# zsyOAOA/ResShift

Hardware: NVIDIA H100
Metric: 256x256 x4 SR images/sec (15 steps), denoising hot path (higher is better)
Workload: dtype f16 (fp32 accumulate)

## Files before the change

resshift_b200/csrc/common.cuh:

```cuda
#pragma once

#include <cuda.h>
#include <cuda_fp16.h>
#include <cuda_runtime.h>
#include <cstdint>
#include <cstdio>
#include <string>

namespace rs {

void set_error(const std::string& msg);
int fail(int code, const std::string& msg);

#define RS_CUDA_OK(expr)                                                                       \
  do {                                                                                         \
    cudaError_t _e = (expr);                                                                   \
    if (_e != cudaSuccess) {                                                                   \
      (void)cudaGetLastError();             \
      return ::rs::fail(-2, std::string(#expr) + " failed: " + cudaGetErrorString(_e) + " (" + \
                                __FILE__ + ":" + std::to_string(__LINE__) + ")");              \
    }                                                                                          \
  } while (0)

#define RS_CHECK(cond, msg)                                                              \
  do {                                                                                   \
    if (!(cond)) {                                                                       \
      return ::rs::fail(-1, std::string("check failed: ") + #cond + " — " + (msg) + " (" + \
                                __FILE__ + ":" + std::to_string(__LINE__) + ")");        \
    }                                                                                    \
  } while (0)

#ifdef __CUDACC__

__device__ __forceinline__ uint32_t smem_u32(const void* p) {
  return static_cast<uint32_t>(__cvta_generic_to_shared(p));
}

__device__ __forceinline__ bool elect_one() {
  uint32_t pred = 0;
  asm volatile(
      "{\n\t"
      ".reg .pred P;\n\t"
      "elect.sync _|P, 0xffffffff;\n\t"
      "selp.u32 %0, 1, 0, P;\n\t"
      "}\n"
      : "=r"(pred));
  return pred != 0;
}

__device__ __forceinline__ void pdl_wait() { asm volatile("griddepcontrol.wait;" ::: "memory"); }
__device__ __forceinline__ void pdl_trigger() { asm volatile("griddepcontrol.launch_dependents;" ::: "memory"); }

__device__ __forceinline__ float silu_f(float v) { return __fdividef(v, 1.0f + __expf(-v)); }
__device__ __forceinline__ float gelu_erf_f(float v) {
  const float z = fminf(fabsf(v) * 0.70710678118654752f, 4.0f);
  float pz = fmaf(z, -2.177763781e-05f, 5.068330793e-04f);
  pz = fmaf(z, pz, -5.339398049e-03f);
  pz = fmaf(z, pz, 3.423144668e-02f);
  pz = fmaf(z, pz, -1.528908461e-01f);
  pz = fmaf(z, pz, -9.167589545e-01f);
  pz = fmaf(z, pz, -1.628154397e+00f);
  pz = fmaf(z, pz, 6.178960575e-06f);
  float ex;
  asm("ex2.approx.ftz.f32 %0, %1;" : "=f"(ex) : "f"(pz));
  const float h = 0.5f * v;
  return h + fmaf(-fabsf(h), ex, fabsf(h));
}

__device__ __forceinline__ void mbar_init(uint64_t* bar, uint32_t count) {
  asm volatile("mbarrier.init.shared::cta.b64 [%0], %1;" ::"r"(smem_u32(bar)), "r"(count));
}
__device__ __forceinline__ void mbar_fence_init() {
  asm volatile("fence.mbarrier_init.release.cluster;" ::: "memory");
}
__device__ __forceinline__ void mbar_arrive_expect_tx(uint64_t* bar, uint32_t bytes) {
  asm volatile("mbarrier.arrive.expect_tx.shared::cta.b64 _, [%0], %1;" ::"r"(smem_u32(bar)), "r"(bytes)
               : "memory");
}
__device__ __forceinline__ void mbar_arrive(uint64_t* bar) {
  asm volatile("mbarrier.arrive.shared::cta.b64 _, [%0];" ::"r"(smem_u32(bar)) : "memory");
}
__device__ __forceinline__ bool mbar_try_wait(uint64_t* bar, uint32_t parity) {
  uint32_t ok;
  asm volatile(
      "{\n\t"
      ".reg .pred P;\n\t"
      "mbarrier.try_wait.parity.shared::cta.b64 P, [%1], %2;\n\t"
      "selp.u32 %0, 1, 0, P;\n\t"
      "}\n"
      : "=r"(ok)
      : "r"(smem_u32(bar)), "r"(parity)
      : "memory");
  return ok != 0;
}
__device__ __forceinline__ void mbar_arrive_remote(uint32_t bar_cluster_addr) {
  asm volatile("mbarrier.arrive.shared::cluster.b64 _, [%0];" ::"r"(bar_cluster_addr) : "memory");
}
__device__ __forceinline__ uint64_t global_timer_ns() {
  uint64_t t;
  asm volatile("mov.u64 %0, %%globaltimer;" : "=l"(t));
  return t;
}
__device__ __forceinline__ void mbar_wait(uint64_t* bar, uint32_t parity) {
  if (mbar_try_wait(bar, parity)) return;
  const uint64_t t0 = global_timer_ns();
  uint32_t spins = 0;
  while (!mbar_try_wait(bar, parity)) {
    if ((++spins & 0xFFu) == 0 && global_timer_ns() - t0 > 2000000000ull) __trap();
  }
}

__device__ __forceinline__ void tma_prefetch_desc(const CUtensorMap* m) {
  asm volatile("prefetch.tensormap [%0];" ::"l"(reinterpret_cast<uint64_t>(m)) : "memory");
}
__device__ __forceinline__ void tma_load_2d(void* dst, const CUtensorMap* m, uint64_t* bar, int c0, int c1) {
  asm volatile(
      "cp.async.bulk.tensor.2d.shared::cluster.global.tile.mbarrier::complete_tx::bytes [%0], [%1, {%3, %4}], [%2];"
      ::"r"(smem_u32(dst)), "l"(reinterpret_cast<uint64_t>(m)), "r"(smem_u32(bar)), "r"(c0), "r"(c1)
      : "memory");
}
__device__ __forceinline__ void tma_load_4d(void* dst, const CUtensorMap* m, uint64_t* bar, int c0, int c1, int c2,
                                            int c3) {
  asm volatile(
      "cp.async.bulk.tensor.4d.shared::cluster.global.tile.mbarrier::complete_tx::bytes [%0], [%1, {%3, %4, %5, %6}], "
      "[%2];" ::"r"(smem_u32(dst)),
      "l"(reinterpret_cast<uint64_t>(m)), "r"(smem_u32(bar)), "r"(c0), "r"(c1), "r"(c2), "r"(c3)
      : "memory");
}

__device__ __forceinline__ uint32_t cluster_ctarank() {
  uint32_t r;
  asm volatile("mov.u32 %0, %%cluster_ctarank;" : "=r"(r));
  return r;
}
__device__ __forceinline__ void cluster_sync_all() {
  asm volatile("barrier.cluster.arrive.release.aligned;" ::: "memory");
  asm volatile("barrier.cluster.wait.acquire.aligned;" ::: "memory");
}
__device__ __forceinline__ uint32_t mapa_u32(uint32_t addr, uint32_t rank) {
  uint32_t r;
  asm volatile("mapa.shared::cluster.u32 %0, %1, %2;" : "=r"(r) : "r"(addr), "r"(rank));
  return r;
}
__device__ __forceinline__ void tma_load_2d_mc(void* dst, const CUtensorMap* m, uint64_t* bar, int c0, int c1, uint16_t cta_mask) {
  asm volatile(
      "cp.async.bulk.tensor.2d.shared::cluster.global.tile.mbarrier::complete_tx::bytes.multicast::cluster [%0], [%1, {%3, %4}], [%2], %5;"
      ::"r"(smem_u32(dst)), "l"(reinterpret_cast<uint64_t>(m)), "r"(smem_u32(bar)), "r"(c0), "r"(c1), "h"(cta_mask)
      : "memory");
}

__device__ __forceinline__ void tma_store_4d(const CUtensorMap* m, const void* src, int c0, int c1, int c2, int c3) {
  asm volatile("cp.async.bulk.tensor.4d.global.shared::cta.tile.bulk_group [%0, {%2, %3, %4, %5}], [%1];" ::"l"(
                   reinterpret_cast<uint64_t>(m)),
               "r"(smem_u32(src)), "r"(c0), "r"(c1), "r"(c2), "r"(c3)
               : "memory");
}
__device__ __forceinline__ void tma_store_commit() { asm volatile("cp.async.bulk.commit_group;" ::: "memory"); }
__device__ __forceinline__ void tma_store_wait_read() { asm volatile("cp.async.bulk.wait_group.read 0;" ::: "memory"); }
__device__ __forceinline__ void tma_store_wait_read_keep1() { asm volatile("cp.async.bulk.wait_group.read 1;" ::: "memory"); }
__device__ __forceinline__ void st_shared_v4(uint32_t addr, uint32_t a, uint32_t b, uint32_t c, uint32_t d) {
  asm volatile("st.shared.v4.b32 [%0], {%1, %2, %3, %4};" ::"r"(addr), "r"(a), "r"(b), "r"(c), "r"(d) : "memory");
}
__device__ __forceinline__ void fence_proxy_async_smem() { asm volatile("fence.proxy.async.shared::cta;" ::: "memory"); }
__device__ __forceinline__ void named_bar_sync(int id, int nthreads) {
  asm volatile("bar.sync %0, %1;" ::"r"(id), "r"(nthreads) : "memory");
}

__device__ __forceinline__ void wgmma_fence() { asm volatile("wgmma.fence.sync.aligned;" ::: "memory"); }
__device__ __forceinline__ void wgmma_commit() { asm volatile("wgmma.commit_group.sync.aligned;" ::: "memory"); }
template <int kPending>
__device__ __forceinline__ void wgmma_wait() { asm volatile("wgmma.wait_group.sync.aligned %0;" ::"n"(kPending) : "memory"); }
template <int kRegs>
__device__ __forceinline__ void wgmma_fence_regs(float (&d)[kRegs]) {
#pragma unroll
  for (int i = 0; i < kRegs; ++i) asm volatile("" : "+f"(d[i])::"memory");
}

__device__ __forceinline__ uint64_t wgmma_desc_sw128(uint32_t smem_addr) {
  uint64_t d = 0;
  d |= static_cast<uint64_t>((smem_addr & 0x3FFFFu) >> 4);
  d |= static_cast<uint64_t>(1) << 16;
  d |= static_cast<uint64_t>(1024 >> 4) << 32;
  d |= static_cast<uint64_t>(1) << 62;
  return d;
}

#endif

}
```

resshift_b200/csrc/gn_stats.cuh:

```cuda
#pragma once

#include "common.cuh"

namespace rs {

struct GnSink {
  float* part;
  float* gstat;
  unsigned int* counter;
  int cstride;
  int coff;
  unsigned int expected;
  float eps;
};

#ifdef __CUDACC__

__device__ __forceinline__ float2 ldcg_f2(const float* p) {
  float2 v;
  asm volatile("ld.global.cg.v2.f32 {%0, %1}, [%2];" : "=f"(v.x), "=f"(v.y) : "l"(p) : "memory");
  return v;
}

__device__ __forceinline__ unsigned int atom_add_acq_rel_gpu(unsigned int* p, unsigned int v) {
  unsigned int old;
  asm volatile("atom.add.acq_rel.gpu.global.u32 %0, [%1], %2;" : "=r"(old) : "l"(p), "r"(v) : "memory");
  return old;
}

__device__ __forceinline__ void chan_merge_equal(float n, float m0, float q0, float m1, float q1, float& m, float& q) {
  m = 0.5f * (m0 + m1);
  const float d0 = m0 - m, d1 = m1 - m;
  q = q0 + q1 + n * (d0 * d0 + d1 * d1);
}

template <int kG>
__device__ __forceinline__ void gn_finalize_groups(const float* part, int n, int slots, int C, int g0, int gstep, int cpg, float ns,
                                                   float eps, float* gstat, int lane) {
  const float* base = part + (size_t)n * slots * C * 2;
  const int K = slots * cpg;
  float pivot[kG], s1[kG], s2[kG];
#pragma unroll
  for (int q = 0; q < kG; ++q) {
    const int g = g0 + q * gstep;
    pivot[q] = g < 32 ? ldcg_f2(base + (size_t)(g * cpg) * 2).x : 0.f;
    s1[q] = 0.f; s2[q] = 0.f;
  }
  for (int i0 = 0; i0 < K; i0 += 128) {
    float2 e[kG][4];
#pragma unroll
    for (int q = 0; q < kG; ++q) {
      const int g = g0 + q * gstep;
#pragma unroll
      for (int u = 0; u < 4; ++u) {
        const int i = i0 + u * 32 + lane;
        if (g < 32 && i < K) {
          const int sl = i / cpg, c = i - sl * cpg;
          e[q][u] = ldcg_f2(base + ((size_t)sl * C + g * cpg + c) * 2);
        } else {
          e[q][u] = make_float2(pivot[q], 0.f);
        }
      }
    }
#pragma unroll
    for (int q = 0; q < kG; ++q)
#pragma unroll
      for (int u = 0; u < 4; ++u) {
        const float d = e[q][u].x - pivot[q];
        s1[q] += d;
        s2[q] += fmaf(ns * d, d, e[q][u].y);
      }
  }
#pragma unroll
  for (int q = 0; q < kG; ++q) {
    float a = s1[q], b = s2[q];
#pragma unroll
    for (int off = 16; off; off >>= 1) {
      a += __shfl_xor_sync(0xffffffffu, a, off);
      b += __shfl_xor_sync(0xffffffffu, b, off);
    }
    const int g = g0 + q * gstep;
    const float invK = 1.0f / (float)K;
    const float dm = a * invK;
    const float m2 = fmaxf(b - ns * (float)K * dm * dm, 0.f);
    const float var = m2 * invK / ns;
    if (lane == 0 && g < 32) {
      gstat[((size_t)n * 32 + g) * 2] = pivot[q] + dm;
      gstat[((size_t)n * 32 + g) * 2 + 1] = rsqrtf(var + eps);
    }
  }
}

template <int kMax>
__device__ __forceinline__ void gn_arrive(const GnSink* const (&sink)[kMax], const int (&img)[kMax], const unsigned int (&add)[kMax],
                                          int slots, float ns, int tid, int nthreads, int bar_id, int* s_flag ) {
  named_bar_sync(bar_id, nthreads);
  if (tid < kMax) {
    int last = 0;
    if (sink[tid] != nullptr && img[tid] >= 0 && sink[tid]->gstat != nullptr) {
      const unsigned int old = atom_add_acq_rel_gpu(sink[tid]->counter + img[tid], add[tid]);
      last = (old + add[tid] == sink[tid]->expected) ? 1 : 0;
    }
    s_flag[tid] = last;
  }
  named_bar_sync(bar_id, nthreads);
  const int warp = tid >> 5, lane = tid & 31, nwarps = nthreads >> 5;
#pragma unroll
  for (int i = 0; i < kMax; ++i) {
    if (!s_flag[i]) continue;
    const GnSink& s = *sink[i];
    const int cpg = s.cstride / 32;
    for (int g = warp; g < 32; g += 4 * nwarps) gn_finalize_groups<4>(s.part, img[i], slots, s.cstride, g, nwarps, cpg, ns, s.eps, s.gstat, lane);
  }
  named_bar_sync(bar_id, nthreads);
}

template <typename Ld>
__device__ __forceinline__ void pivot_stats2(Ld ld, int rows, float2& mean, float2& m2) {
  const float2 p = ld(0);
  float2 s1 = make_float2(0.f, 0.f), s2 = make_float2(0.f, 0.f);
  for (int r = 1; r < rows; ++r) {
    const float2 v = ld(r);
    const float dx = v.x - p.x, dy = v.y - p.y;
    s1.x += dx; s1.y += dy;
    s2.x = fmaf(dx, dx, s2.x); s2.y = fmaf(dy, dy, s2.y);
  }
  const float inv = 1.0f / (float)rows;
  mean = make_float2(p.x + s1.x * inv, p.y + s1.y * inv);
  m2 = make_float2(fmaxf(s2.x - s1.x * s1.x * inv, 0.f), fmaxf(s2.y - s1.y * s1.y * inv, 0.f));
}

__device__ __forceinline__ void warp_chunk_stats(const uint4& o0, const uint4& o1, int lane, float* dst) {
  float sv[16], sq[16];
  const __half2* q0 = reinterpret_cast<const __half2*>(&o0);
  const __half2* q1 = reinterpret_cast<const __half2*>(&o1);
#pragma unroll
  for (int j = 0; j < 4; ++j) {
    const float2 x0 = __half22float2(q0[j]);
    const float2 x1 = __half22float2(q1[j]);
    sv[2 * j] = x0.x; sv[2 * j + 1] = x0.y; sv[8 + 2 * j] = x1.x; sv[8 + 2 * j + 1] = x1.y;
  }
#pragma unroll
  for (int j = 0; j < 16; ++j) sq[j] = sv[j] * sv[j];
#pragma unroll
  for (int half = 8, bit = 16; half >= 1; half >>= 1, bit >>= 1) {
    const bool upper = (lane & bit) != 0;
#pragma unroll
    for (int j = 0; j < half; ++j) {
      const float send_s = upper ? sv[j] : sv[j + half];
      const float keep_s = upper ? sv[j + half] : sv[j];
      sv[j] = keep_s + __shfl_xor_sync(0xffffffffu, send_s, bit);
      const float send_q = upper ? sq[j] : sq[j + half];
      const float keep_q = upper ? sq[j + half] : sq[j];
      sq[j] = keep_q + __shfl_xor_sync(0xffffffffu, send_q, bit);
    }
  }
  sv[0] += __shfl_xor_sync(0xffffffffu, sv[0], 1);
  sq[0] += __shfl_xor_sync(0xffffffffu, sq[0], 1);
  if ((lane & 1) == 0) {
    const int cidx = ((lane >> 4) & 1) * 8 + ((lane >> 3) & 1) * 4 + ((lane >> 2) & 1) * 2 + ((lane >> 1) & 1);
    const float mean = sv[0] * (1.0f / 32.0f);
    dst[cidx * 2] = mean;
    dst[cidx * 2 + 1] = fmaxf(sq[0] - sv[0] * mean, 0.f);
  }
}

__device__ __forceinline__ void write_quad_pairs(const float* wq, int BN, int ncols, int col0, int bn, int n0, int Nimg, int slot,
                                                 int slots, const GnSink& s0, const GnSink& s1, int tid, int nthreads) {
  for (int cc = tid; cc < ncols; cc += nthreads) {
    float m[4], q[4];
#pragma unroll
    for (int k = 0; k < 4; ++k) { m[k] = wq[((size_t)k * BN + cc) * 2]; q[k] = wq[((size_t)k * BN + cc) * 2 + 1]; }
    float ma, qa, mb, qb;
    chan_merge_equal(32.f, m[0], q[0], m[1], q[1], ma, qa);
    chan_merge_equal(32.f, m[2], q[2], m[3], q[3], mb, qb);
#pragma unroll
    for (int d = 0; d < 2; ++d) {
      const GnSink& s = d == 0 ? s0 : s1;
      if (!s.part) continue;
      const size_t ch = (size_t)s.coff + col0 + cc;
      float* dst = s.part + (((size_t)n0 * slots + slot) * s.cstride + ch) * 2;
      if (bn == 1) {
        float mm, qq;
        chan_merge_equal(64.f, ma, qa, mb, qb, mm, qq);
        dst[0] = mm; dst[1] = qq;
      } else {
        dst[0] = ma; dst[1] = qa;
        if (n0 + 1 < Nimg) {
          float* dst1 = s.part + (((size_t)(n0 + 1) * slots + slot) * s.cstride + ch) * 2;
          dst1[0] = mb; dst1[1] = qb;
        }
      }
    }
  }
}

__device__ __forceinline__ float2 gn_channel_from_pairs(const float* part_nc , int slots, int C, float ns) {
  const float pivot = reinterpret_cast<const float2*>(part_nc)->x;
  float s1 = 0.f, s2 = 0.f;
  int sl = 0;
  for (; sl + 16 <= slots; sl += 16) {
    float2 e[16];
#pragma unroll
    for (int u = 0; u < 16; ++u) e[u] = *reinterpret_cast<const float2*>(part_nc + (size_t)(sl + u) * C * 2);
#pragma unroll
    for (int u = 0; u < 16; ++u) { const float d = e[u].x - pivot; s1 += d; s2 += fmaf(ns * d, d, e[u].y); }
  }
  for (; sl + 4 <= slots; sl += 4) {
    float2 e[4];
#pragma unroll
    for (int u = 0; u < 4; ++u) e[u] = *reinterpret_cast<const float2*>(part_nc + (size_t)(sl + u) * C * 2);
#pragma unroll
    for (int u = 0; u < 4; ++u) { const float d = e[u].x - pivot; s1 += d; s2 += fmaf(ns * d, d, e[u].y); }
  }
  for (; sl < slots; ++sl) {
    const float2 e = *reinterpret_cast<const float2*>(part_nc + (size_t)sl * C * 2);
    const float d = e.x - pivot; s1 += d; s2 += fmaf(ns * d, d, e.y);
  }
  const float dm = s1 / (float)slots;
  return make_float2(pivot + dm, fmaxf(s2 - ns * (float)slots * dm * dm, 0.f));
}
__device__ __forceinline__ float2 gn_group_from_channels(const float* ch_pairs , int cpg, float cnt, float eps) {
  const float pivot = ch_pairs[0];
  float s1 = 0.f, s2 = 0.f;
  for (int j = 0; j < cpg; ++j) { const float d = ch_pairs[2 * j] - pivot; s1 += d; s2 += fmaf(cnt * d, d, ch_pairs[2 * j + 1]); }
  const float dm = s1 / (float)cpg;
  const float m2 = fmaxf(s2 - cnt * (float)cpg * dm * dm, 0.f);
  return make_float2(pivot + dm, rsqrtf(m2 / (cnt * (float)cpg) + eps));
}

#endif
}
```

resshift_b200/csrc/launch.cuh:

```cuda
#pragma once

#include <algorithm>
#include <atomic>
#include <cstdlib>
#include <cmath>
#include <cstring>
#include <mutex>
#include <utility>
#include <vector>

#include "common.cuh"
#include "conv_gemm.cuh"
#include "elementwise.cuh"
#include "mlp_fused.cuh"
#include "norm_act.cuh"
#include "window_attn.cuh"
#include "swin_attn_fused.cuh"
#include "vq_attn.cuh"
#include "unet_attn.cuh"

namespace rs {

typedef CUresult (*PFN_encodeTiled)(CUtensorMap*, CUtensorMapDataType, cuuint32_t, void*, const cuuint64_t*,
                                    const cuuint64_t*, const cuuint32_t*, const cuuint32_t*, CUtensorMapInterleave,
// ... 464 lines not shown
    RS_CUDA_OK(cudaFuncSetAttribute(unet_attn_sm90_kernel<128>, cudaFuncAttributeMaxDynamicSharedMemorySize, UnetAttnSmem<128>::launch_bytes));
    attr_set[dev].store(true, std::memory_order_release);
  }
  return 0;
}

inline int conv_launch(const ConvDesc& d, cudaStream_t st) {
  if (d.simt_kernel) {
    const long long npix = (long long)d.prm.Nimg * d.prm.Hout * d.prm.Wout;
    const int warps = 8;
    (void)launch_k(conv_simt_kernel, dim3((unsigned)((npix + warps - 1) / warps)), dim3(warps * 32), (size_t)(0), st, d.prm, d.simt);
  } else {
    const ConvKernelFn k = conv_kernel_for(d.prm.BN, d.prm.msub, d.has_silu || d.film);
    RS_CHECK(k != nullptr, "no conv kernel for this channel tile");
    (void)launch_kc(k, dim3(d.grid), dim3(kConvThreads), (size_t)(d.smem), st, d.prm.cg, d.prm);
    if (d.prm.splitk > 1)
      (void)launch_k(splitk_reduce_kernel, dim3(d.red_grid_x, d.prm.Nimg, d.red_grid_z), dim3(256), d.red_smem, st, d.red);
  }
  RS_CUDA_OK(cudaGetLastError());
  return 0;
}

inline int conv_tile_slots(int H, int W, bool* fusable = nullptr) {
  const int bw = pow2_floor_div(W, kConvBM);
  const int bh = pow2_floor_div(H, kConvBM / bw);
  if (fusable) *fusable = (kConvBM / (bw * bh)) <= 2;
  return (W / bw) * (H / bh);
}

struct GnDesc {
  View in, out;
  const float* gamma = nullptr; const float* beta = nullptr;
  const float* film = nullptr; long long film_sN = 0;
  int film_off = -1;
  int silu = 0;
  float* part = nullptr;
  float* gstat = nullptr;
  unsigned int* counter = nullptr;
  float eps = 1e-5f;
  int slots = 0;
  bool fused = false;
  bool finalize_kernel = false;
};

inline void gn_chunks(int HW, int N, int* chunks, int* rows) {
  int c = std::max(1, std::min((HW + 31) / 32, (num_sms() * 4 + N - 1) / N));
  while (c > 1 && HW % c != 0) --c;
  *chunks = c; *rows = HW / c;
}

struct GnGeometry {
  int slots = 0;
  int rows_per_slot = 0;
  int stats_ctas = 0;
  bool finalize = false;
  int apply_ctas = 0;
  int apply_rows = 0;
  int csplit = 1;
};

inline GnGeometry gn_geometry(const GnDesc& g) {
  const int C = g.in.C, HW = g.in.H * g.in.W, N = g.in.N;
  GnGeometry r;
  r.slots = g.slots;
  if (!g.fused) {
    int chunks, rows;
    gn_chunks(HW, N, &chunks, &rows);
    if (r.slots <= 0) r.slots = chunks;
    r.stats_ctas = r.slots;
  }
  r.rows_per_slot = r.slots > 0 ? HW / r.slots : 0;
  r.finalize = g.fused && g.finalize_kernel;
  int actas = std::max(1, std::min((HW + 15) / 16, (num_sms() * 4 + N - 1) / N));
  r.apply_rows = (HW + actas - 1) / actas;
  r.apply_ctas = (HW + r.apply_rows - 1) / r.apply_rows;
  const int cpg = C / 32;
  int unit = cpg; while (unit % 8) unit += cpg;
  for (int cs = 2; r.apply_ctas * N * r.csplit < num_sms() * 3 / 2 && cs <= C / unit; ++cs)
    if (C % cs == 0 && (C / cs) % unit == 0) r.csplit = cs;
  return r;
}

inline int gn_launch(const GnDesc& g, cudaStream_t st) {
  const int C = g.in.C, HW = g.in.H * g.in.W, N = g.in.N;
  RS_CHECK(C % 32 == 0 && C % 8 == 0 && C <= 2048, "GroupNorm channel count");
  RS_CHECK(g.in.ld % 8 == 0 && g.out.ld % 8 == 0, "GroupNorm view alignment");
  RS_CHECK(g.gstat != nullptr || g.part != nullptr, "GroupNorm needs a statistics buffer");
  const GnGeometry geo = gn_geometry(g);
  const int slots = geo.slots;
  if (!g.fused) {
    const int lanes = 256 / (C / 8);
    RS_CHECK(g.part != nullptr && (g.gstat == nullptr || g.counter != nullptr), "GroupNorm statistics buffers");
    RS_CHECK(HW % slots == 0, "GroupNorm statistics slots must divide H*W");
    GnStatsParams sp{};
    sp.x = g.in.ptr; sp.sN = g.in.sN(); sp.ld = g.in.ld; sp.C = C; sp.HW = HW; sp.N = N;
    sp.sink.part = g.part; sp.sink.gstat = g.gstat; sp.sink.counter = g.counter; sp.sink.cstride = C; sp.sink.coff = 0;
    sp.sink.expected = (unsigned)(slots * C); sp.sink.eps = g.eps;
    sp.slots = slots; sp.rows_per_slot = geo.rows_per_slot;
    (void)launch_k(gn_stats_kernel, dim3(geo.stats_ctas, N), dim3(256), (size_t)lanes * C * 3 * sizeof(float) + 16, st, sp);
    RS_CUDA_OK(cudaGetLastError());
  }
  if (geo.finalize) {
    RS_CHECK(g.part != nullptr && g.gstat != nullptr && slots > 0 && HW % slots == 0, "GroupNorm finalisation buffers");
    GnFinalizeParams fp{g.part, g.gstat, slots, C, (float)geo.rows_per_slot, g.eps};
    (void)launch_k(gn_finalize_kernel, dim3(32, N), dim3(256), (size_t)0, st, fp);
    RS_CUDA_OK(cudaGetLastError());
  }
  GnApplyParams ap{g.in.ptr, g.in.sN(), g.in.ld, g.out.ptr, g.out.sN(), g.out.ld, C, HW, N, g.gstat, g.part, slots, g.eps,
                   g.gamma, g.beta, g.film, g.film_sN, g.silu, geo.apply_rows, C / geo.csplit};
  (void)launch_k(gn_apply_kernel, dim3(geo.apply_ctas, N, geo.csplit), dim3(256),
                 (size_t)(4 * (C / geo.csplit) + 64) * sizeof(float), st, ap);
  RS_CUDA_OK(cudaGetLastError());
  return 0;
}

struct MlpDesc {
  View in, out, res;
  bool has_res = true;
  const __half* w1 = nullptr; const float* b1 = nullptr;
  const __half* w2 = nullptr; const float* b2 = nullptr;
  int E = 0, Hd = 0;
  GnSink sink[2] = {};
  MlpParams prm;
  int grid = 0; size_t smem = 0;
};

inline bool mlp_supported(int E, int Hd, int H, int W, int N) {
  (void)N;
  bool fus = false;
  conv_tile_slots(H, W, &fus);
  return (E == 64 || E == 128 || E == 192 || E == 256) && Hd % kMlpHc == 0 && fus;
}

inline int mlp_finalize(MlpDesc& d) {
  MlpParams& p = d.prm;
  std::memset(&p, 0, sizeof(p));
  const int H = d.in.H, W = d.in.W, N = d.in.N;
  RS_CHECK(mlp_supported(d.E, d.Hd, H, W, N), "fused MLP: unsupported shape (E in {64, 128, 192, 256}, hidden % 64)");
  RS_CHECK(d.in.C == d.E && d.out.C == d.E, "fused MLP: channel mismatch");
  p.E = d.E; p.Hd = d.Hd; p.bias1 = d.b1; p.bias2 = d.b2;
  p.bw = pow2_floor_div(W, kConvBM);
  p.bh = pow2_floor_div(H, kConvBM / p.bw);
  p.bn = kConvBM / (p.bw * p.bh);
  p.tiles_w = W / p.bw; p.tiles_h = H / p.bh;
  const int tiles_n = (N + p.bn - 1) / p.bn;
  p.Wout = W; p.Hout = H; p.Nimg = N;
  const int slot = std::max(kMlpHc, d.E) * kConvBK * 2;
  const int fixed = MlpSmem(d.E, d.Hd, 0).total + 1024;
  p.ring = std::min(8, (227 * 1024 - fixed) / slot);
  RS_CHECK(p.ring >= 2, "fused MLP: not enough shared memory for the weight ring");
  d.smem = (size_t)MlpSmem(d.E, d.Hd, p.ring).total + 1024;
  RS_CHECK(d.smem <= 227 * 1024, "fused MLP: shared memory budget exceeded");
  p.has_res = d.has_res ? 1 : 0;
  d.grid = p.tiles_w * p.tiles_h * tiles_n;
  int rc = encode_act_map(&p.tmX, d.in.ptr, d.E, W, H, N, d.in.sW(), d.in.sH(), d.in.sN(), p.bw, p.bh, p.bn, 64);
  if (rc) return rc;
  rc = encode_weight_map(&p.tmW1, d.w1, d.E, d.Hd, kMlpHc); if (rc) return rc;
  rc = encode_weight_map(&p.tmW2, d.w2, d.Hd, d.E, d.E); if (rc) return rc;
  rc = encode_act_map(&p.tmOut, d.out.ptr, d.E, W, H, N, d.out.sW(), d.out.sH(), d.out.sN(), p.bw, p.bh, p.bn, 64);
  if (rc) return rc;
  if (d.has_res) {
    rc = encode_act_map(&p.tmRes, d.res.ptr, d.E, W, H, N, d.res.sW(), d.res.sH(), d.res.sN(), p.bw, p.bh, p.bn, 64);
    if (rc) return rc;
  }
  p.gn_slots = p.tiles_w * p.tiles_h;
  compact_sinks(d.sink, p.gn_slots, p.sink);
  return 0;
}

inline int mlp_launch(const MlpDesc& d, cudaStream_t st) {
  switch (d.E) {
    case 64: (void)launch_k(mlp_fused_sm90_kernel<64>, dim3(d.grid), dim3(kMlpThreads), d.smem, st, d.prm); break;
    case 128: (void)launch_k(mlp_fused_sm90_kernel<128>, dim3(d.grid), dim3(kMlpThreads), d.smem, st, d.prm); break;
    case 192: (void)launch_k(mlp_fused_sm90_kernel<192>, dim3(d.grid), dim3(kMlpThreads), d.smem, st, d.prm); break;
    case 256: (void)launch_k(mlp_fused_sm90_kernel<256>, dim3(d.grid), dim3(kMlpThreads), d.smem, st, d.prm); break;
    default: RS_CHECK(false, "fused MLP: embedding width");
  }
  RS_CUDA_OK(cudaGetLastError());
  return 0;
}

struct SwinAttnDesc {
  View x, y;
  int heads = 0, shift = 0;
  const float* gn_part = nullptr; int gn_slots = 0; const float* gn_gstat = nullptr;
  const float* gamma = nullptr; const float* beta = nullptr;
  const __half* wqkv = nullptr; int wqkv_ld = 0; const float* bqkv = nullptr;
  const float* relbias = nullptr;
  const __half* wproj = nullptr; int wproj_ld = 0; const float* bproj = nullptr;
  GnSink sink[2] = {};
  SwinAttnParams prm;
  GnFinalizeParams fin[2] = {};
  int grid = 0;
};
inline bool swin_attn_supported(int E, int heads, int H, int W, int window) {
  return window == 8 && (E == 192 || E == 64) && heads * 32 == E && H % 8 == 0 && W % 8 == 0;
}
inline int swin_attn_finalize(SwinAttnDesc& d) {
  SwinAttnParams& p = d.prm;
  std::memset(&p, 0, sizeof(p));
  const int E = d.x.C;
  RS_CHECK(swin_attn_supported(E, d.heads, d.x.H, d.x.W, 8), "fused Swin attention: E in {64, 192}, head_dim 32, H and W multiples of 8");
  RS_CHECK(d.y.C == E && d.y.H == d.x.H && d.y.W == d.x.W && d.y.N == d.x.N, "fused Swin attention: output geometry");
  RS_CHECK(d.x.ld % 8 == 0 && d.y.ld % 8 == 0 && d.wqkv_ld % 8 == 0 && d.wproj_ld % 8 == 0, "fused Swin attention: 16-byte rows");
  RS_CHECK((d.gn_part && d.gn_slots > 0) || d.gn_gstat, "fused Swin attention: norm1 statistics");
  int rc = encode_weight_map(&p.tmWqkv, d.wqkv, d.wqkv_ld, 3 * E, 64); if (rc) return rc;
  rc = encode_weight_map(&p.tmWproj, d.wproj, d.wproj_ld, E, 64); if (rc) return rc;
  p.x = d.x.ptr; p.x_ld = d.x.ld; p.y = d.y.ptr; p.y_ld = d.y.ld;
  p.N = d.x.N; p.H = d.x.H; p.W = d.x.W; p.heads = d.heads; p.shift = d.shift; p.scale = 0.17677669529663687f;
  p.gn_part = d.gn_part; p.gn_slots = d.gn_slots; p.gn_gstat = d.gn_gstat; p.gamma = d.gamma; p.beta = d.beta; p.eps = 1e-5f;
  p.wqkv = d.wqkv; p.wqkv_ld = d.wqkv_ld; p.bqkv = d.bqkv; p.relbias = d.relbias;
  p.wproj = d.wproj; p.wproj_ld = d.wproj_ld; p.bproj = d.bproj;
  p.total_windows = d.x.N * (d.x.H / 8) * (d.x.W / 8);
  const int nW = (d.x.H / 8) * (d.x.W / 8);
  compact_sinks(d.sink, nW, p.sink);
  const int pairs = (p.total_windows + 1) / 2;
  d.grid = std::min(pairs, num_sms());
  for (int k = 0; k < 2; ++k) {
    d.fin[k] = GnFinalizeParams{};
    if (p.sink[k].gstat) {
      RS_CHECK(p.sink[k].coff == 0 && p.sink[k].cstride == E, "fused Swin attention: group statistics of a channel slice");
      d.fin[k] = GnFinalizeParams{p.sink[k].part, p.sink[k].gstat, nW, E, 64.0f, p.sink[k].eps};
    }
    p.sink[k].gstat = nullptr; p.sink[k].counter = nullptr;
  }
  return 0;
}
inline int swin_attn_launch(const SwinAttnDesc& d, cudaStream_t st) {
  if (d.x.C == 192) (void)launch_k(swin_attn_fused_kernel<192>, dim3(d.grid), dim3(kSwinThreads), (size_t)SwinSmem<192>::launch_bytes, st, d.prm);
  else (void)launch_k(swin_attn_fused_kernel<64>, dim3(d.grid), dim3(kSwinThreads), (size_t)SwinSmem<64>::launch_bytes, st, d.prm);
  RS_CUDA_OK(cudaGetLastError());
  for (int k = 0; k < 2; ++k)
    if (d.fin[k].gstat) {
      (void)launch_k(gn_finalize_kernel, dim3(32, d.x.N), dim3(256), (size_t)0, st, d.fin[k]);
      RS_CUDA_OK(cudaGetLastError());
    }
  return 0;
}

struct VqAttnDesc {
  View q, k, v, out;
  int row_begin = 0, row_end = -1;
  VqAttnParams prm;
};
inline int vq_attn_set_rows(VqAttnDesc& d, long long row_begin, long long row_end, bool allow_empty) {
  const long long T = (long long)d.q.H * d.q.W;
  RS_CHECK(row_begin >= 0 && row_begin <= row_end && row_end <= T,
           "fused VQ-GAN attention: rows [" + std::to_string(row_begin) + ", " + std::to_string(row_end) + ") outside [0, T = " + std::to_string(T) + ")");
  RS_CHECK(row_begin % kVqAttnBM == 0 && row_end % kVqAttnBM == 0, "fused VQ-GAN attention: row range bounds must be multiples of 64");
  RS_CHECK(allow_empty || row_end > row_begin, "fused VQ-GAN attention: empty row range");
  d.row_begin = (int)row_begin; d.row_end = (int)row_end;
  d.prm.q_tile0 = (int)(row_begin / kVqAttnBM);
  return 0;
}
inline int vq_attn_finalize(VqAttnDesc& d) {
  VqAttnParams& p = d.prm;
  std::memset(&p, 0, sizeof(p));
  const int N = d.q.N, C = d.q.C;
  const long long T = (long long)d.q.H * d.q.W;
  RS_CHECK(C == 128 || C == 256 || C == 512, "fused VQ-GAN attention: C in {128, 256, 512}, got " + std::to_string(C));
  RS_CHECK(T > 0 && T % kVqAttnBM == 0 && T <= (1LL << 30), "fused VQ-GAN attention: T = H * W must be a positive multiple of 64, got " + std::to_string(T));
  RS_CHECK(N >= 1 && N <= 65535, "fused VQ-GAN attention: batch in [1, 65535]");
  const View* vs[4] = {&d.q, &d.k, &d.v, &d.out};
  for (const View* v : vs) {
    RS_CHECK(v->N == N && (long long)v->H * v->W == T && v->C == C, "fused VQ-GAN attention: q, k, v, out must all be [N, T, C]");
    RS_CHECK(v->ptr != nullptr && v->ld >= C && v->ld % 8 == 0, "fused VQ-GAN attention: rows of >= C elements, 16-byte aligned");
  }
  p.T = (int)T;
  { int rc = vq_attn_set_rows(d, d.row_begin, d.row_end < 0 ? T : d.row_end, true); if (rc) return rc; }
  p.scale_log2 = (float)(1.4426950408889634 / std::sqrt((double)C));
  CUtensorMap* maps[4] = {&p.tmQ, &p.tmK, &p.tmV, &p.tmO};
  const int rows[4] = {kVqAttnBM, vq_attn_bk(C), vq_attn_bk(C), kVqAttnBM};
  for (int i = 0; i < 4; ++i) {
    const View& v = *vs[i];
    int rc = encode_act_map(maps[i], v.ptr, C, (int)T, 1, N, v.ld, T * v.ld, v.sN(), rows[i], 1, 1, 64);
    if (rc) return rc;
  }
  return 0;
}
inline int vq_attn_launch(const VqAttnDesc& d, cudaStream_t st) {
  if (d.row_end == d.row_begin) return 0;
  const dim3 grid((unsigned)((d.row_end - d.row_begin) / kVqAttnBM), (unsigned)d.q.N);
  switch (d.q.C) {
    case 128: (void)launch_k(vq_attn_sm90_kernel<128>, grid, dim3(kVqAttnThreads), (size_t)VqAttnSmem<128>::launch_bytes, st, d.prm); break;
    case 256: (void)launch_k(vq_attn_sm90_kernel<256>, grid, dim3(kVqAttnThreads), (size_t)VqAttnSmem<256>::launch_bytes, st, d.prm); break;
    case 512: (void)launch_k(vq_attn_sm90_kernel<512>, grid, dim3(kVqAttnThreads), (size_t)VqAttnSmem<512>::launch_bytes, st, d.prm); break;
    default: RS_CHECK(false, "fused VQ-GAN attention: C in {128, 256, 512}");
  }
  RS_CUDA_OK(cudaGetLastError());
  return 0;
}

struct UnetAttnDesc {
  View qkv, out;
  int heads = 1;
  bool new_order = false;
  UnetAttnParams prm;
};
inline bool unet_attn_head_dim_ok(int D) { return D == 32 || D == 64 || D == 128; }
inline int unet_attn_finalize(UnetAttnDesc& d) {
  UnetAttnParams& p = d.prm;
  std::memset(&p, 0, sizeof(p));
  const int N = d.qkv.N, C = d.out.C;
  const long long T = (long long)d.qkv.H * d.qkv.W;
  RS_CHECK(d.heads > 0 && C % d.heads == 0 && unet_attn_head_dim_ok(C / d.heads),
           "UNetModel attention: head dim (channels / heads) must be 32, 64 or 128");
  const int D = C / d.heads;
  RS_CHECK(d.qkv.C == 3 * C && d.out.N == N && (long long)d.out.H * d.out.W == T, "UNetModel attention: qkv [N, T, 3C] -> out [N, T, C]");
  RS_CHECK(T >= 1 && T <= (1LL << 30) && N >= 1 && N <= 65535 && d.heads <= 65535, "UNetModel attention: T >= 1, batch and heads <= 65535");
  RS_CHECK(d.qkv.ptr && d.out.ptr && d.qkv.ld % 8 == 0 && d.out.ld % 2 == 0 && d.out.ld >= C, "UNetModel attention: views");
  p.out = d.out.ptr; p.out_sN = d.out.sN(); p.out_ld = d.out.ld;
  p.T = (int)T;
  p.head_stride = d.new_order ? D : 3 * D;
  p.k_col0 = d.new_order ? C : D;
  p.v_col0 = d.new_order ? 2 * C : 2 * D;
  p.scale_log2 = (float)(1.4426950408889634 / std::sqrt((double)D));
  return encode_act_map(&p.tm, d.qkv.ptr, 3 * C, (int)T, 1, N, d.qkv.ld, T * d.qkv.ld, d.qkv.sN(), kUnetAttnBK, 1, 1, 64);
}
inline int unet_attn_launch(const UnetAttnDesc& d, cudaStream_t st) {
  const long long T = (long long)d.qkv.H * d.qkv.W;
  const dim3 grid((unsigned)((T + kUnetAttnCtaRows - 1) / kUnetAttnCtaRows), (unsigned)d.heads, (unsigned)d.qkv.N);
  switch (d.out.C / d.heads) {
    case 32: (void)launch_k(unet_attn_sm90_kernel<32>, grid, dim3(kUnetAttnThreads), (size_t)UnetAttnSmem<32>::launch_bytes, st, d.prm); break;
    case 64: (void)launch_k(unet_attn_sm90_kernel<64>, grid, dim3(kUnetAttnThreads), (size_t)UnetAttnSmem<64>::launch_bytes, st, d.prm); break;
    case 128: (void)launch_k(unet_attn_sm90_kernel<128>, grid, dim3(kUnetAttnThreads), (size_t)UnetAttnSmem<128>::launch_bytes, st, d.prm); break;
    default: RS_CHECK(false, "UNetModel attention: head dim 32, 64 or 128");
  }
  RS_CUDA_OK(cudaGetLastError());
// ... 43 lines not shown
```

resshift_b200/csrc/mlp_fused.cuh:

```cuda
#pragma once

#include "common.cuh"
#include "conv_gemm.cuh"

namespace rs {

constexpr int kMlpHc = 64;
constexpr int kMlpThreads = kConvThreads;
constexpr int kMlpTmaWarp = kConvTmaWarp;

struct MlpParams {
  CUtensorMap tmX, tmW1, tmW2, tmOut, tmRes;
  const float* bias1;
  const float* bias2;
  int E, Hd;
  int ring;
  int bw, bh, bn, tiles_w, tiles_h;
  int Wout, Hout, Nimg;
  int has_res;
  GnSink sink[2]; int gn_slots;
};

struct MlpSmem {
  int x, h, ring, bars, b1, b2, total;
  __host__ __device__ MlpSmem(int E, int Hd, int ring_depth) {
    const int slot = (E > kMlpHc ? E : kMlpHc) * kConvBK * 2;
    x = 0;
    h = x + (E / 64) * kConvBM * kConvBK * 2;
    ring = h + (kMlpHc / 64) * kConvBM * kConvBK * 2;
    bars = ring + ring_depth * slot;
    b1 = bars + 1024;
    b2 = b1 + Hd * 4;
    total = b2 + E * 4;
  }
};

#ifdef __CUDACC__

template <int E>
__global__ void __launch_bounds__(kMlpThreads, 1) mlp_fused_sm90_kernel(const __grid_constant__ MlpParams p) {
  extern __shared__ __align__(1024) uint8_t smem_raw[];
  uint8_t* smem = reinterpret_cast<uint8_t*>((reinterpret_cast<uintptr_t>(smem_raw) + 1023) & ~uintptr_t(1023));
  constexpr int kx = E / 64;
  constexpr int kTile = kConvBM * kConvBK * 2;
  constexpr int kW1 = kMlpHc * kConvBK * 2;
  constexpr int kW2 = E * kConvBK * 2;
  constexpr int kSlot = kW1 > kW2 ? kW1 : kW2;
  const MlpSmem L(E, p.Hd, p.ring);
  uint8_t* sX = smem + L.x;
  uint8_t* sH = smem + L.h;
  uint8_t* sRing = smem + L.ring;
  uint64_t* full_bar = reinterpret_cast<uint64_t*>(smem + L.bars);
  uint64_t* empty_bar = full_bar + p.ring;
  uint64_t* x_full = empty_bar + p.ring;
  uint64_t* res_bar = x_full + 1;
  float* s_b1 = reinterpret_cast<float*>(smem + L.b1);
  float* s_b2 = reinterpret_cast<float*>(smem + L.b2);

  const int warp = threadIdx.x >> 5, lane = threadIdx.x & 31;
  const int chunks = p.Hd / kMlpHc;
  int mt = (int)blockIdx.x;
  const int tw = mt % p.tiles_w; mt /= p.tiles_w;
  const int th = mt % p.tiles_h; mt /= p.tiles_h;
  const int w0 = tw * p.bw, h0 = th * p.bh, n0 = mt * p.bn;

  if (warp == kMlpTmaWarp && lane == 0) {
    tma_prefetch_desc(&p.tmX); tma_prefetch_desc(&p.tmW1); tma_prefetch_desc(&p.tmW2);
    tma_prefetch_desc(&p.tmOut); if (p.has_res) tma_prefetch_desc(&p.tmRes);
    for (int s = 0; s < p.ring; ++s) { mbar_init(&full_bar[s], 1); mbar_init(&empty_bar[s], kConvEpiWarps); }
    mbar_init(x_full, 1); mbar_init(res_bar, 1);
    mbar_fence_init();
  }
  __syncthreads();
  pdl_trigger();
  pdl_wait();

  if (warp == kMlpTmaWarp) {
    const bool el = elect_one();
    if (el) {
      mbar_arrive_expect_tx(x_full, (uint32_t)(kx * kTile));
      for (int kb = 0; kb < kx; ++kb) tma_load_4d(sX + (size_t)kb * kTile, &p.tmX, x_full, kb * kConvBK, w0, h0, n0);
    }
    int stage = 0; uint32_t phase = 0;
    auto next = [&]() { if (++stage == p.ring) { stage = 0; phase ^= 1; } };
    for (int j = 0; j < chunks; ++j) {
      for (int kb = 0; kb < kx; ++kb) {
        mbar_wait(&empty_bar[stage], phase ^ 1);
        if (el) {
          mbar_arrive_expect_tx(&full_bar[stage], (uint32_t)kW1);
          tma_load_2d(sRing + (size_t)stage * kSlot, &p.tmW1, &full_bar[stage], kb * kConvBK, j * kMlpHc);
        }
        next();
      }
      for (int t = 0; t < kMlpHc / kConvBK; ++t) {
        mbar_wait(&empty_bar[stage], phase ^ 1);
        if (el) {
          mbar_arrive_expect_tx(&full_bar[stage], (uint32_t)kW2);
          tma_load_2d(sRing + (size_t)stage * kSlot, &p.tmW2, &full_bar[stage], j * kMlpHc + t * kConvBK, 0);
        }
        next();
      }
    }
    return;
  }

  const int wg = warp >> 2;
  const int rA = 64 * wg + 16 * (warp & 3) + (lane >> 2), rB = rA + 8;
  const int etid = threadIdx.x;
  constexpr int kCons = 32 * kConvEpiWarps;
  for (int i = etid; i < p.Hd; i += kCons) s_b1[i] = __ldg(p.bias1 + i);
  for (int i = etid; i < E; i += kCons) s_b2[i] = __ldg(p.bias2 + i);
  mbar_wait(x_full, 0);
  named_bar_sync(1, kCons);

  const uint32_t sX0 = smem_u32(sX), sH0 = smem_u32(sH), sR0 = smem_u32(sRing);
  int stage = 0; uint32_t phase = 0;
  auto release = [&](int s) { if (s >= 0 && lane == 0) mbar_arrive(&empty_bar[s]); };
  float acc2[E / 2];
#pragma unroll
  for (int i = 0; i < E / 2; ++i) acc2[i] = 0.f;
  for (int j = 0; j < chunks; ++j) {
    float acc1[kMlpHc / 2];
#pragma unroll
    for (int i = 0; i < kMlpHc / 2; ++i) acc1[i] = 0.f;
    int prev = -1;
    for (int kb = 0; kb < kx; ++kb) {
      mbar_wait(&full_bar[stage], phase);
      const uint64_t adesc = wgmma_desc_sw128(sX0 + (uint32_t)(kb * kTile + wg * (64 * 128)));
      const uint64_t bdesc = wgmma_desc_sw128(sR0 + (uint32_t)(stage * kSlot));
      wgmma_fence();
#pragma unroll
      for (int k = 0; k < kConvBK / 16; ++k) Wgmma<kMlpHc>::mma(acc1, adesc + 2 * k, bdesc + 2 * k);
      wgmma_commit();
      wgmma_wait<1>();
      release(prev);
      prev = stage;
      if (++stage == p.ring) { stage = 0; phase ^= 1; }
    }
    wgmma_wait<0>();
    wgmma_fence_regs(acc1);
    release(prev);
    const float* b1 = s_b1 + j * kMlpHc;
#pragma unroll
    for (int i = 0; i < kMlpHc / 8; ++i) {
      const int c = 8 * i + 2 * (lane & 3);
      const float2 bb = *reinterpret_cast<const float2*>(b1 + c);
      uint8_t* tile = sH + (size_t)(c >> 6) * kTile + 4 * (lane & 3);
      const int u = (c & 63) >> 3;
#pragma unroll
      for (int hr = 0; hr < 2; ++hr) {
        const int r = hr ? rB : rA;
        *reinterpret_cast<__half2*>(tile + r * 128 + ((u ^ (r & 7)) << 4)) =
            __floats2half2_rn(gelu_erf_f(acc1[4 * i + 2 * hr] + bb.x), gelu_erf_f(acc1[4 * i + 2 * hr + 1] + bb.y));
      }
    }
    fence_proxy_async_smem();
    named_bar_sync(2 + wg, 128);
    prev = -1;
    for (int t = 0; t < kMlpHc / kConvBK; ++t) {
      mbar_wait(&full_bar[stage], phase);
      const uint64_t adesc = wgmma_desc_sw128(sH0 + (uint32_t)(t * kTile + wg * (64 * 128)));
      const uint64_t bdesc = wgmma_desc_sw128(sR0 + (uint32_t)(stage * kSlot));
      wgmma_fence();
#pragma unroll
      for (int k = 0; k < kConvBK / 16; ++k) Wgmma<E>::mma(acc2, adesc + 2 * k, bdesc + 2 * k);
      wgmma_commit();
      wgmma_wait<1>();
      release(prev);
      prev = stage;
      if (++stage == p.ring) { stage = 0; phase ^= 1; }
    }
    wgmma_wait<0>();
    wgmma_fence_regs(acc2);
    release(prev);
  }

  named_bar_sync(1, kCons);
  uint8_t* sblk = sX;
  float* wsum = reinterpret_cast<float*>(sH);
  if (p.has_res) {
    if (etid == 0) {
      mbar_arrive_expect_tx(res_bar, (uint32_t)(kx * kTile));
      for (int bq = 0; bq < kx; ++bq) tma_load_4d(sblk + (size_t)bq * kTile, &p.tmRes, res_bar, bq * 64, w0, h0, n0);
    }
    mbar_wait(res_bar, 0);
  }
#pragma unroll
  for (int i = 0; i < E / 8; ++i) {
    const int c = 8 * i + 2 * (lane & 3);
    const float2 bb = *reinterpret_cast<const float2*>(s_b2 + c);
    uint8_t* tile = sblk + (size_t)(c >> 6) * kTile + 4 * (lane & 3);
    const int u = (c & 63) >> 3;
#pragma unroll
    for (int hr = 0; hr < 2; ++hr) {
      const int r = hr ? rB : rA;
      __half2* dst = reinterpret_cast<__half2*>(tile + r * 128 + ((u ^ (r & 7)) << 4));
      float f0 = acc2[4 * i + 2 * hr] + bb.x, f1 = acc2[4 * i + 2 * hr + 1] + bb.y;
      if (p.has_res) { const float2 x = __half22float2(*dst); f0 += x.x; f1 += x.y; }
      *dst = __floats2half2_rn(f0, f1);
    }
  }
  named_bar_sync(1, kCons);
  const bool want_stats = p.sink[0].part != nullptr;
  if (want_stats) {
    const int quad = warp & 3, cpar = warp >> 2;
    const int r = quad * 32 + lane;
    for (int c = cpar * 16; c < E; c += 32) {
      const uint8_t* brow = sblk + (size_t)(c >> 6) * kTile + r * 128;
      const int u0 = (c & 63) >> 3;
      const uint4 o0 = *reinterpret_cast<const uint4*>(brow + (((u0) ^ (r & 7)) << 4));
      const uint4 o1 = *reinterpret_cast<const uint4*>(brow + (((u0 + 1) ^ (r & 7)) << 4));
      warp_chunk_stats(o0, o1, lane, wsum + ((size_t)quad * E + c) * 2);
    }
  }
  fence_proxy_async_smem();
  named_bar_sync(1, kCons);
  if (etid == 0) {
    for (int bq = 0; bq < kx; ++bq) tma_store_4d(&p.tmOut, sblk + (size_t)bq * kTile, bq * 64, w0, h0, n0);
    tma_store_commit();
  }
  if (want_stats) {
    const int slot = th * p.tiles_w + tw;
    if (n0 < p.Nimg)
      write_quad_pairs(wsum, E, E, 0, p.bn, n0, p.Nimg, slot, p.gn_slots, p.sink[0], p.sink[1], etid, kCons);
    if (p.sink[0].gstat || p.sink[1].gstat) {
      int* s_flag = reinterpret_cast<int*>(wsum + 8 * E);
      const GnSink* const sk[4] = {&p.sink[0], &p.sink[0], p.sink[1].part ? &p.sink[1] : nullptr, p.sink[1].part ? &p.sink[1] : nullptr};
      const int n1 = (p.bn == 2 && n0 + 1 < p.Nimg) ? n0 + 1 : -1;
      const int im[4] = {n0 < p.Nimg ? n0 : -1, n0 < p.Nimg ? n1 : -1, n0 < p.Nimg ? n0 : -1, n0 < p.Nimg ? n1 : -1};
      const unsigned int ad[4] = {(unsigned)E, (unsigned)E, (unsigned)E, (unsigned)E};
      gn_arrive<4>(sk, im, ad, p.gn_slots, 128.0f / (float)p.bn, etid, kCons, 1, s_flag);
    }
  }
  if (etid == 0) tma_store_wait_read();
}

#endif
}
```

Measured before the change: 137.3.

## Split fused MLP hidden dimension across cluster CTAs with DSMEM reduction

New measurement: 165.4 (median of 6 runs). 20.5% higher.

```diff
diff --git a/resshift_b200/csrc/common.cuh b/resshift_b200/csrc/common.cuh
--- a/resshift_b200/csrc/common.cuh
+++ b/resshift_b200/csrc/common.cuh
@@ -142,6 +142,11 @@
   asm volatile("mapa.shared::cluster.u32 %0, %1, %2;" : "=r"(r) : "r"(addr), "r"(rank));
   return r;
 }
+__device__ __forceinline__ float2 ld_dsmem_f32x2(uint32_t addr) {
+  float2 v;
+  asm volatile("ld.shared::cluster.v2.f32 {%0, %1}, [%2];" : "=f"(v.x), "=f"(v.y) : "r"(addr) : "memory");
+  return v;
+}
 __device__ __forceinline__ void tma_load_2d_mc(void* dst, const CUtensorMap* m, uint64_t* bar, int c0, int c1, uint16_t cta_mask) {
   asm volatile(
       "cp.async.bulk.tensor.2d.shared::cluster.global.tile.mbarrier::complete_tx::bytes.multicast::cluster [%0], [%1, {%3, %4}], [%2], %5;"
@@ -164,6 +169,9 @@
 __device__ __forceinline__ void fence_proxy_async_smem() { asm volatile("fence.proxy.async.shared::cta;" ::: "memory"); }
 __device__ __forceinline__ void named_bar_sync(int id, int nthreads) {
   asm volatile("bar.sync %0, %1;" ::"r"(id), "r"(nthreads) : "memory");
+}
+__device__ __forceinline__ void named_bar_arrive(int id, int nthreads) {
+  asm volatile("bar.arrive %0, %1;" ::"r"(id), "r"(nthreads) : "memory");
 }
 
 __device__ __forceinline__ void wgmma_fence() { asm volatile("wgmma.fence.sync.aligned;" ::: "memory"); }
diff --git a/resshift_b200/csrc/gn_stats.cuh b/resshift_b200/csrc/gn_stats.cuh
--- a/resshift_b200/csrc/gn_stats.cuh
+++ b/resshift_b200/csrc/gn_stats.cuh
@@ -130,6 +130,21 @@
   m2 = make_float2(fmaxf(s2.x - s1.x * s1.x * inv, 0.f), fmaxf(s2.y - s1.y * s1.y * inv, 0.f));
 }
 
+template <int kHalf>
+__device__ __forceinline__ void warp_xor_step(float (&sv)[16], float (&sq)[16], int lane) {
+  constexpr int bit = 2 * kHalf;
+  const bool upper = (lane & bit) != 0;
+#pragma unroll
+  for (int j = 0; j < kHalf; ++j) {
+    const float send_s = upper ? sv[j] : sv[j + kHalf];
+    const float keep_s = upper ? sv[j + kHalf] : sv[j];
+    sv[j] = keep_s + __shfl_xor_sync(0xffffffffu, send_s, bit);
+    const float send_q = upper ? sq[j] : sq[j + kHalf];
+    const float keep_q = upper ? sq[j + kHalf] : sq[j];
+    sq[j] = keep_q + __shfl_xor_sync(0xffffffffu, send_q, bit);
+  }
+}
+
 __device__ __forceinline__ void warp_chunk_stats(const uint4& o0, const uint4& o1, int lane, float* dst) {
   float sv[16], sq[16];
   const __half2* q0 = reinterpret_cast<const __half2*>(&o0);
@@ -142,19 +157,10 @@
   }
 #pragma unroll
   for (int j = 0; j < 16; ++j) sq[j] = sv[j] * sv[j];
-#pragma unroll
-  for (int half = 8, bit = 16; half >= 1; half >>= 1, bit >>= 1) {
-    const bool upper = (lane & bit) != 0;
-#pragma unroll
-    for (int j = 0; j < half; ++j) {
-      const float send_s = upper ? sv[j] : sv[j + half];
-      const float keep_s = upper ? sv[j + half] : sv[j];
-      sv[j] = keep_s + __shfl_xor_sync(0xffffffffu, send_s, bit);
-      const float send_q = upper ? sq[j] : sq[j + half];
-      const float keep_q = upper ? sq[j + half] : sq[j];
-      sq[j] = keep_q + __shfl_xor_sync(0xffffffffu, send_q, bit);
-    }
-  }
+  warp_xor_step<8>(sv, sq, lane);
+  warp_xor_step<4>(sv, sq, lane);
+  warp_xor_step<2>(sv, sq, lane);
+  warp_xor_step<1>(sv, sq, lane);
   sv[0] += __shfl_xor_sync(0xffffffffu, sv[0], 1);
   sq[0] += __shfl_xor_sync(0xffffffffu, sq[0], 1);
   if ((lane & 1) == 0) {
diff --git a/resshift_b200/csrc/launch.cuh b/resshift_b200/csrc/launch.cuh
--- a/resshift_b200/csrc/launch.cuh
+++ b/resshift_b200/csrc/launch.cuh
@@ -640,7 +640,12 @@
   d.smem = (size_t)MlpSmem(d.E, d.Hd, p.ring).total + 1024;
   RS_CHECK(d.smem <= 227 * 1024, "fused MLP: shared memory budget exceeded");
   p.has_res = d.has_res ? 1 : 0;
-  d.grid = p.tiles_w * p.tiles_h * tiles_n;
+  const int tiles = p.tiles_w * p.tiles_h * tiles_n, chunks = d.Hd / kMlpHc;
+  p.split = 1;
+  if (p.ring * slot >= kConvBM * d.E * 4)
+    for (int s = 2; s <= 4 && tiles * p.split < num_sms() / 2; ++s)
+      if (chunks % s == 0) p.split = s;
+  d.grid = tiles * p.split;
   int rc = encode_act_map(&p.tmX, d.in.ptr, d.E, W, H, N, d.in.sW(), d.in.sH(), d.in.sN(), p.bw, p.bh, p.bn, 64);
   if (rc) return rc;
   rc = encode_weight_map(&p.tmW1, d.w1, d.E, d.Hd, kMlpHc); if (rc) return rc;
@@ -658,10 +663,10 @@
 
 inline int mlp_launch(const MlpDesc& d, cudaStream_t st) {
   switch (d.E) {
-    case 64: (void)launch_k(mlp_fused_sm90_kernel<64>, dim3(d.grid), dim3(kMlpThreads), d.smem, st, d.prm); break;
-    case 128: (void)launch_k(mlp_fused_sm90_kernel<128>, dim3(d.grid), dim3(kMlpThreads), d.smem, st, d.prm); break;
-    case 192: (void)launch_k(mlp_fused_sm90_kernel<192>, dim3(d.grid), dim3(kMlpThreads), d.smem, st, d.prm); break;
-    case 256: (void)launch_k(mlp_fused_sm90_kernel<256>, dim3(d.grid), dim3(kMlpThreads), d.smem, st, d.prm); break;
+    case 64: (void)launch_kc(mlp_fused_sm90_kernel<64>, dim3(d.grid), dim3(kMlpThreads), d.smem, st, d.prm.split, d.prm); break;
+    case 128: (void)launch_kc(mlp_fused_sm90_kernel<128>, dim3(d.grid), dim3(kMlpThreads), d.smem, st, d.prm.split, d.prm); break;
+    case 192: (void)launch_kc(mlp_fused_sm90_kernel<192>, dim3(d.grid), dim3(kMlpThreads), d.smem, st, d.prm.split, d.prm); break;
+    case 256: (void)launch_kc(mlp_fused_sm90_kernel<256>, dim3(d.grid), dim3(kMlpThreads), d.smem, st, d.prm.split, d.prm); break;
     default: RS_CHECK(false, "fused MLP: embedding width");
   }
   RS_CUDA_OK(cudaGetLastError());
diff --git a/resshift_b200/csrc/mlp_fused.cuh b/resshift_b200/csrc/mlp_fused.cuh
--- a/resshift_b200/csrc/mlp_fused.cuh
+++ b/resshift_b200/csrc/mlp_fused.cuh
@@ -18,13 +18,14 @@
   int bw, bh, bn, tiles_w, tiles_h;
   int Wout, Hout, Nimg;
   int has_res;
+  int split;
   GnSink sink[2]; int gn_slots;
 };
 
 struct MlpSmem {
   int x, h, ring, bars, b1, b2, total;
   __host__ __device__ MlpSmem(int E, int Hd, int ring_depth) {
-    const int slot = (E > kMlpHc ? E : kMlpHc) * kConvBK * 2;
+    const int slot = E * kConvBK * 2;
     x = 0;
     h = x + (E / 64) * kConvBM * kConvBK * 2;
     ring = h + (kMlpHc / 64) * kConvBM * kConvBK * 2;
@@ -45,7 +46,8 @@
   constexpr int kTile = kConvBM * kConvBK * 2;
   constexpr int kW1 = kMlpHc * kConvBK * 2;
   constexpr int kW2 = E * kConvBK * 2;
-  constexpr int kSlot = kW1 > kW2 ? kW1 : kW2;
+  constexpr int kSlot = kx * kW1;
+  static_assert(kSlot == kW2 && kMlpHc == kConvBK, "one fc1 slot and one fc2 slot per hidden chunk");
   const MlpSmem L(E, p.Hd, p.ring);
   uint8_t* sX = smem + L.x;
   uint8_t* sH = smem + L.h;
@@ -58,8 +60,11 @@
   float* s_b2 = reinterpret_cast<float*>(smem + L.b2);
 
   const int warp = threadIdx.x >> 5, lane = threadIdx.x & 31;
-  const int chunks = p.Hd / kMlpHc;
-  int mt = (int)blockIdx.x;
+  const int split = p.split;
+  const int rank = (int)blockIdx.x % split;
+  const int chunks = p.Hd / kMlpHc / split;
+  const int j0 = rank * chunks;
+  int mt = (int)blockIdx.x / split;
   const int tw = mt % p.tiles_w; mt /= p.tiles_w;
   const int th = mt % p.tiles_h; mt /= p.tiles_h;
   const int w0 = tw * p.bw, h0 = th * p.bh, n0 = mt * p.bn;
@@ -83,24 +88,23 @@
     }
     int stage = 0; uint32_t phase = 0;
     auto next = [&]() { if (++stage == p.ring) { stage = 0; phase ^= 1; } };
-    for (int j = 0; j < chunks; ++j) {
-      for (int kb = 0; kb < kx; ++kb) {
-        mbar_wait(&empty_bar[stage], phase ^ 1);
-        if (el) {
-          mbar_arrive_expect_tx(&full_bar[stage], (uint32_t)kW1);
-          tma_load_2d(sRing + (size_t)stage * kSlot, &p.tmW1, &full_bar[stage], kb * kConvBK, j * kMlpHc);
-        }
-        next();
-      }
-      for (int t = 0; t < kMlpHc / kConvBK; ++t) {
-        mbar_wait(&empty_bar[stage], phase ^ 1);
-        if (el) {
-          mbar_arrive_expect_tx(&full_bar[stage], (uint32_t)kW2);
-          tma_load_2d(sRing + (size_t)stage * kSlot, &p.tmW2, &full_bar[stage], j * kMlpHc + t * kConvBK, 0);
-        }
-        next();
-      }
-    }
+    for (int j = j0; j < j0 + chunks; ++j) {
+      mbar_wait(&empty_bar[stage], phase ^ 1);
+      if (el) {
+        mbar_arrive_expect_tx(&full_bar[stage], (uint32_t)(kx * kW1));
+        for (int kb = 0; kb < kx; ++kb)
+          tma_load_2d(sRing + (size_t)stage * kSlot + (size_t)kb * kW1, &p.tmW1, &full_bar[stage], kb * kConvBK, j * kMlpHc);
+      }
+      next();
+      mbar_wait(&empty_bar[stage], phase ^ 1);
+      if (el) {
+        mbar_arrive_expect_tx(&full_bar[stage], (uint32_t)kW2);
+        tma_load_2d(sRing + (size_t)stage * kSlot, &p.tmW2, &full_bar[stage], j * kMlpHc, 0);
+      }
+      next();
+    }
+    __syncwarp();
+    if (split > 1) { cluster_sync_all(); cluster_sync_all(); }
     return;
   }
 
@@ -115,32 +119,45 @@
 
   const uint32_t sX0 = smem_u32(sX), sH0 = smem_u32(sH), sR0 = smem_u32(sRing);
   int stage = 0; uint32_t phase = 0;
+  auto take = [&]() { mbar_wait(&full_bar[stage], phase); const int s = stage; if (++stage == p.ring) { stage = 0; phase ^= 1; } return s; };
   auto release = [&](int s) { if (s >= 0 && lane == 0) mbar_arrive(&empty_bar[s]); };
+  constexpr int kTurn = 2;
   float acc2[E / 2];
 #pragma unroll
   for (int i = 0; i < E / 2; ++i) acc2[i] = 0.f;
+  auto gemm2 = [&]() {
+    const int s = take();
+    const uint64_t adesc = wgmma_desc_sw128(sH0 + (uint32_t)(wg * (64 * 128)));
+    const uint64_t bdesc = wgmma_desc_sw128(sR0 + (uint32_t)(s * kSlot));
+    wgmma_fence();
+#pragma unroll
+    for (int k = 0; k < kConvBK / 16; ++k) Wgmma<E>::mma(acc2, adesc + 2 * k, bdesc + 2 * k);
+    wgmma_commit();
+    return s;
+  };
   for (int j = 0; j < chunks; ++j) {
     float acc1[kMlpHc / 2];
 #pragma unroll
     for (int i = 0; i < kMlpHc / 2; ++i) acc1[i] = 0.f;
-    int prev = -1;
+    if (wg == 1 || j > 0) named_bar_sync(kTurn + wg, 256);
+    const int s2 = j > 0 ? gemm2() : -1;
+    const int s1 = take();
+    wgmma_fence();
+#pragma unroll
     for (int kb = 0; kb < kx; ++kb) {
-      mbar_wait(&full_bar[stage], phase);
       const uint64_t adesc = wgmma_desc_sw128(sX0 + (uint32_t)(kb * kTile + wg * (64 * 128)));
-      const uint64_t bdesc = wgmma_desc_sw128(sR0 + (uint32_t)(stage * kSlot));
-      wgmma_fence();
+      const uint64_t bdesc = wgmma_desc_sw128(sR0 + (uint32_t)(s1 * kSlot + kb * kW1));
 #pragma unroll
       for (int k = 0; k < kConvBK / 16; ++k) Wgmma<kMlpHc>::mma(acc1, adesc + 2 * k, bdesc + 2 * k);
-      wgmma_commit();
-      wgmma_wait<1>();
-      release(prev);
-      prev = stage;
-      if (++stage == p.ring) { stage = 0; phase ^= 1; }
-    }
+    }
+    wgmma_commit();
+    named_bar_arrive(kTurn + 1 - wg, 256);
     wgmma_wait<0>();
     wgmma_fence_regs(acc1);
-    release(prev);
-    const float* b1 = s_b1 + j * kMlpHc;
+    wgmma_fence_regs(acc2);
+    release(s2);
+    release(s1);
+    const float* b1 = s_b1 + (j0 + j) * kMlpHc;
 #pragma unroll
     for (int i = 0; i < kMlpHc / 8; ++i) {
       const int c = 8 * i + 2 * (lane & 3);
@@ -155,27 +172,38 @@
       }
     }
     fence_proxy_async_smem();
-    named_bar_sync(2 + wg, 128);
-    prev = -1;
-    for (int t = 0; t < kMlpHc / kConvBK; ++t) {
-      mbar_wait(&full_bar[stage], phase);
-      const uint64_t adesc = wgmma_desc_sw128(sH0 + (uint32_t)(t * kTile + wg * (64 * 128)));
-      const uint64_t bdesc = wgmma_desc_sw128(sR0 + (uint32_t)(stage * kSlot));
-      wgmma_fence();
-#pragma unroll
-      for (int k = 0; k < kConvBK / 16; ++k) Wgmma<E>::mma(acc2, adesc + 2 * k, bdesc + 2 * k);
-      wgmma_commit();
-      wgmma_wait<1>();
-      release(prev);
-      prev = stage;
-      if (++stage == p.ring) { stage = 0; phase ^= 1; }
-    }
-    wgmma_wait<0>();
-    wgmma_fence_regs(acc2);
-    release(prev);
-  }
-
-  named_bar_sync(1, kCons);
+  }
+  named_bar_sync(kTurn + wg, 256);
+  const int s2 = gemm2();
+  if (wg == 0) named_bar_arrive(kTurn + 1, 256);
+  wgmma_wait<0>();
+  wgmma_fence_regs(acc2);
+  release(s2);
+
+  named_bar_sync(1, kCons);
+  if (split > 1) {
+    const uint32_t red = sR0 + (uint32_t)etid * 8u;
+    if (rank != 0) {
+      float2* mine = reinterpret_cast<float2*>(sRing) + etid;
+#pragma unroll
+      for (int i = 0; i < E / 4; ++i) mine[i * kCons] = make_float2(acc2[2 * i], acc2[2 * i + 1]);
+    }
+    cluster_sync_all();
+    if (rank == 0) {
+      for (int r = 1; r < split; ++r) {
+        const uint32_t base = mapa_u32(red, (uint32_t)r);
+#pragma unroll
+        for (int i = 0; i < E / 4; ++i) {
+          const float2 v = ld_dsmem_f32x2(base + (uint32_t)(i * kCons * 8));
+          acc2[2 * i] += v.x;
+          acc2[2 * i + 1] += v.y;
+        }
+      }
+    }
+    cluster_sync_all();
+    if (rank != 0) return;
+  }
+
   uint8_t* sblk = sX;
   float* wsum = reinterpret_cast<float*>(sH);
   if (p.has_res) {
```
